# dusk-network/dusk-blindbidproof

Measured on AMD Instinct MI355X. Metric: blind-bid proofs/sec, higher is better.
Workload: dtype u32

## Files before the change

dusk_blindbidproof_amd/csrc/capi_prove.hip:

```cpp
#include <stdio.h>
#include <string.h>
#include <unistd.h>

#include <algorithm>
#include <chrono>
#include <functional>
#include <thread>

#include "batch.h"
#include "chacha.h"
#include "round_bids.h"
#include "submit.h"
#include "witness_check.h"

namespace bbp {
int32_t prove_batch_dev(bbp_ctx* ctx, u32 B, u32 N, const u8* in_dev, const u8* ent_dev, u8* out_dev, hipStream_t s,
                        const std::function<int32_t(hipStream_t)>* open_hook = nullptr);
int32_t verify_batch_dev(bbp_ctx* ctx, const VerifyRows& v, u32 G, const u8* in_dev, const u8* ent_dev, int32_t* status_dev, hipStream_t s);
int32_t verify_batch_agg_dev(bbp_ctx* ctx, const VerifyRows& v, u32 G, const u8* in_dev, const u8* ent_dev, int32_t* status_dev, hipStream_t s,
                             u32* n_fallback, u32* total_out_dev = nullptr);
int32_t debug_read_misc(bbp_ctx* ctx, u32 B, u32 N, u32 proof, uint8_t* out);
int32_t debug_varbase(bbp_ctx* ctx, u32 form, u32 B, u32 Q, u32 agg, const u32* ns, const u8* vers, const u8* pts, const u8* scal, const u8* wv,
                      const u8* uj, u8* sums_out, u32* digits_out, int32_t* status_out);
int32_t round_consts_launch(bbp_ctx* ctx, u32 N, const u8* round_dev, const u32* roff_dev, sc* rblk, int32_t* rflag, hipStream_t s);
// ... 1338 lines not shown
                rcs[i] = bbp_reserve(ctx->members[i], max_batch, N);
            }
        }
        for (auto& t : th) t.join();
        for (int32_t r : rcs)
            if (r) return r;
        return BBP_OK;
    }
    return no_throw_ctx(ctx, [&]() -> int32_t {
        const uint32_t B = max_batch;
        const VerifyRows vrows = VerifyRows::uniform(B, N);
        std::vector<uint8_t> in(prove_in_bytes(N) * B, 0), ent(entropy_row_bytes(N) * B, 0), out(proof_record_bytes(N) * B), vin(vrows.row_bytes(0) * B, 0);
        std::vector<int32_t> st(B);
        int32_t rc = BBP_OK;
        for (int k = 0; k < bbp_ctx::IO_SLOTS && rc == BBP_OK; k++) rc = prove_batch_host(ctx, B, N, in.data(), ent.data(), out.data(), st.data(), CHECK_OFF);
        const uint32_t small = B < 1023 ? B : 1023;
        for (int k = 0; k < bbp_ctx::PROVE_BUFS && rc == BBP_OK; k++) rc = prove_batch_host(ctx, small, N, in.data(), ent.data(), out.data(), st.data(), CHECK_OFF);
        if (B >= 1024 && ctx->knobs.deep_eligible(B)) {
            struct Reset { bool& b; ~Reset() { b = false; } } reset{ctx->prove_state.force_deep};
            ctx->prove_state.force_deep = true;
            for (int k = 0; k < bbp_ctx::PROVE_BUFS && rc == BBP_OK; k++) rc = prove_batch_host(ctx, B, N, in.data(), ent.data(), out.data(), st.data(), CHECK_OFF);
        }
        for (int k = 0; k < bbp_ctx::IO_VSLOTS && rc == BBP_OK; k++) rc = verify_batch_host(ctx, vrows, vin.data(), st.data());
        const bool check = ctx->prove_check;
        for (int k = 0; check && k < bbp_ctx::IO_VSLOTS && rc == BBP_OK; k++) rc = verify_batch_host(ctx, vrows, vin.data(), st.data(), BBP_AGG_GROUP_DEFAULT);
        if (rc == BBP_OK)
            rc = api_guard(ctx, [&]() -> int32_t {
                int32_t rc = BBP_OK;
                BBP_HIP_TRY(ctx, hipSetDevice(ctx->device));
                for (int k = 0; k < bbp_ctx::IO_SLOTS && rc == BBP_OK; k++)
                    if (!(rc = staging_reserve(ctx, ctx->io[k], ProveStaging(B, N, true, check, false)))) rc = staging_reserve(ctx, ctx->io[k], ProveStaging(B, N, false, check, false));
                for (int k = 0; k < bbp_ctx::CHECK_RING && rc == BBP_OK; k++)
                    if (!(rc = dev_reserve(ctx, ctx->rnd[k].buf, RoundRing(B, N, true).bytes)) && check) rc = dev_reserve(ctx, ctx->chk[k].buf, CheckRing(B, N).bytes);
                return rc;
            });
        return rc;
    });
}

extern "C" int32_t bbp_set_batching(bbp_ctx* ctx, uint32_t window_us, uint32_t max_batch) {
    if (!ctx || !ctx->combiner) return BBP_ERR_BAD_ARG;
    return no_throw([&]() -> int32_t {
        static_cast<Combiner*>(ctx->combiner)->configure(window_us, max_batch);
        return BBP_OK;
    });
}

extern "C" int32_t bbp_set_verify_mixing(bbp_ctx* ctx, int32_t on) {
    if (!ctx || !ctx->combiner) return BBP_ERR_BAD_ARG;
    return no_throw([&]() -> int32_t {
        static_cast<Combiner*>(ctx->combiner)->set_verify_mixing(on != 0);
        return BBP_OK;
    });
}

extern "C" int32_t bbp_set_verify_round_sharing(bbp_ctx* ctx, int32_t on) {
    if (!ctx || !ctx->combiner) return BBP_ERR_BAD_ARG;
    return no_throw([&]() -> int32_t {
        static_cast<Combiner*>(ctx->combiner)->set_round_sharing(on != 0);
        return BBP_OK;
    });
}

extern "C" int32_t bbp_verify_round_sharing_stats(bbp_ctx* ctx, uint64_t* n_calls, uint64_t* n_rows, uint64_t* n_rounds) {
    if (!ctx || !ctx->combiner) return BBP_ERR_BAD_ARG;
    return no_throw([&]() -> int32_t {
// ... 105 lines not shown
```

dusk_blindbidproof_amd/csrc/context.h:

```cpp
#pragma once
#include <hip/hip_runtime.h>
#include <stdint.h>
#include <stdio.h>
#include <stdlib.h>
#include <string.h>

#include <atomic>
#include <condition_variable>
#include <map>
#include <mutex>
#include <new>
#include <stdexcept>
#include <string>
#include <vector>

#include "../../include/bbp.h"
#include "point.h"
#include "msm_plan.h"
#include "prove_io.h"
#include "prove_plan.h"
#include "scalar.h"
#include "verify_rows.h"

namespace bbp {
// ... 100 lines not shown
            size_t cap = 0;
            hipEvent_t ev = nullptr;
        };
        std::vector<NsStage> ns_ring;
        uint32_t ns_oldest = 0;
    };
    VLane vl[VLANES];
    std::string err;
    bbp::u32* health = nullptr;
    std::atomic<int> prove_check{0};
    std::atomic<uint64_t> chk_checked{0}, chk_reproved{0};
    unsigned long long* chk_counts = nullptr;
    int64_t debug_corrupt_proof = -1;
    uint32_t chk_lane = 0;
    hipEvent_t ev_chk_fork = nullptr, ev_chk_join = nullptr;
    static constexpr int CHECK_RING = PROVE_BUFS;
    struct CheckBuf {
        bbp::DevBuf buf;
        hipEvent_t ev = nullptr;
        bool ev_valid = false;
    };
    CheckBuf chk[CHECK_RING];
    uint32_t chk_next = 0;
    CheckBuf rnd[CHECK_RING];
    uint32_t rnd_next = 0;
    hipEvent_t ev_round = nullptr;
    bbp::ge* gens = nullptr;
    bbp::niels_row* ptable = nullptr;
    bbp::ge* btab = nullptr;
    bbp::niels_packed* comb = nullptr;
    bbp::sc* mimc_c = nullptr;
    uint8_t gens_enc_host_valid = 0;
    std::vector<uint8_t> mimc_host;
    bbp::DevBuf scal, idx, sorted, pts, enc, batch[PROVE_BUFS + VLANES], io_in, io_out, io_ent, raw[2];
    static constexpr int VERIFY_SLOT = MAX_SLICES;
    bbp::DevBuf slice_sorted[MAX_SLICES + VLANES], slice_pts[MAX_SLICES + VLANES], slice_fold[MAX_SLICES], slice_vtab[MAX_SLICES];
    struct IoSlot {
        bbp::DevBuf in, ent, out, chk;
        uint32_t* h_flag = nullptr;
        void *h_out = nullptr, *h_in = nullptr;
        size_t h_cap = 0, h_in_cap = 0;
        hipEvent_t ev = nullptr, ev_in = nullptr;
        bool busy = false;
    };
    static constexpr int IO_SLOTS = 3;
    static constexpr int IO_VSLOTS = VLANES;
    IoSlot io[IO_SLOTS + IO_VSLOTS];
    std::mutex io_mu;
    std::condition_variable io_cv;
    uint32_t io_next = 0, io_vnext = 0;
    std::map<uint32_t, void*> circuits;
    void* vctab = nullptr;
    uint8_t vctab_has[256] = {};
    std::map<uint64_t, bbp::u32*> layout_idx;
    std::vector<float> timings;
    uint64_t scratch_allocs = 0;
    size_t scratch_bytes = 0;
    bool profile = false;
    struct Ev {
        int tag;
        hipEvent_t a, b;
    };
    std::vector<Ev> events;
};

namespace bbp {

// ... 180 lines not shown
```

dusk_blindbidproof_amd/csrc/prove_plan.h:

```cpp
#pragma once
#include <stdint.h>
#include <stdio.h>
#include <stdlib.h>
#include <string.h>

#include <string>

namespace bbp {

constexpr int FOLD_ROUND = 7;
constexpr int PROVE_MAX_SLICES = 4;
#ifndef BBP_PROVE_BUFS
#define BBP_PROVE_BUFS 5
#endif
constexpr int PROVE_BUFS = BBP_PROVE_BUFS;

struct ProveKnobs {
    int slices = 3;
    int rotate_below = 1023;
    int rotate_deep_max = 4096;
    int deep_from = 3;
    int mixed_from = 512;
    int dual_open_below = 1024;
    int rng_coop = -1;
    int rng_coop_below = 768;
    int rng_coop_idle_below = 2300;
    int rng_dpp = 2;
    int rng_block = 0;
    int serial_block = 64;
    int serial_lds = 160 * 1024;
    int tr_wave_below = 32;
    int ipa_wide_below = 32;
    int commit_split_below = 1024;
    int witness_native = 1;
    int tail_small_below = 65;
    int tail_round = FOLD_ROUND;
    int stagger_mode = 0;
    int trace_prove = 0;

    struct Env {
        const char* name;
        int ProveKnobs::*member;
        int (*clamp)(int);
    };
    template <class F>
    static void each_env(F&& f) {
        static const Env table[] = {
            {"BBP_SLICES", &ProveKnobs::slices, [](int v) { return v < 1 ? 1 : v > PROVE_MAX_SLICES ? PROVE_MAX_SLICES : v; }},
            {"BBP_ROTATE_BELOW", &ProveKnobs::rotate_below, nullptr},
            {"BBP_ROTATE_DEEP_MAX", &ProveKnobs::rotate_deep_max, nullptr},
            {"BBP_ROTATE_DEEP_FROM", &ProveKnobs::deep_from, [](int v) { return v < 2 ? 2 : v; }},
            {"BBP_ROTATE_MIXED_FROM", &ProveKnobs::mixed_from, nullptr},
            {"BBP_DUAL_OPEN_BELOW", &ProveKnobs::dual_open_below, nullptr},
            {"BBP_RNG_COOP", &ProveKnobs::rng_coop, [](int v) { return v != 0 ? 1 : 0; }},
            {"BBP_RNG_COOP_BELOW", &ProveKnobs::rng_coop_below, nullptr},
            {"BBP_RNG_COOP_IDLE_BELOW", &ProveKnobs::rng_coop_idle_below, nullptr},
            {"BBP_RNG_DPP", &ProveKnobs::rng_dpp, nullptr},
            {"BBP_RNG_BLOCK", &ProveKnobs::rng_block, [](int v) { return v >= 1024 ? 1024 : v >= 512 ? 512 : v >= 256 ? 256 : v >= 128 ? 128 : 64; }},
            {"BBP_SERIAL_BLOCK", &ProveKnobs::serial_block, [](int v) { return v == 64 ? 64 : v == 128 ? 128 : 256; }},
            {"BBP_SERIAL_LDS", &ProveKnobs::serial_lds, [](int v) { return v < 0 ? 0 : v > 160 * 1024 ? 160 * 1024 : v; }},
            {"BBP_TR_WAVE_BELOW", &ProveKnobs::tr_wave_below, nullptr},
            {"BBP_IPA_WIDE_BELOW", &ProveKnobs::ipa_wide_below, nullptr},
            {"BBP_COMMIT_SPLIT_BELOW", &ProveKnobs::commit_split_below, nullptr},
            {"BBP_WITNESS_NATIVE", &ProveKnobs::witness_native, [](int v) { return v != 0 ? 1 : 0; }},
            {"BBP_TAIL_SMALL_BELOW", &ProveKnobs::tail_small_below, nullptr},
            {"BBP_TAIL_ROUND", &ProveKnobs::tail_round, [](int v) { return v == FOLD_ROUND ? FOLD_ROUND : 12; }},
            {"BBP_STAGGER", &ProveKnobs::stagger_mode, nullptr},
            {"BBP_TRACE_PROVE", &ProveKnobs::trace_prove, [](int) { return 1; }},
        };
        for (const Env& e : table) f(e);
    }
    bool set(const char* name, const char* text) {
        bool found = false;
        each_env([&](const Env& e) {
            if (strcmp(e.name, name)) return;
            this->*e.member = e.clamp ? e.clamp(atoi(text)) : atoi(text);
            found = true;
        });
        return found;
    }
    static ProveKnobs from_env() {
        ProveKnobs k;
        each_env([&](const Env& e) {
            if (const char* text = getenv(e.name)) k.set(e.name, text);
        });
        return k;
    }

    bool deep_eligible(uint32_t B) const { return slices > 1 && rotate_deep_max > 0 && B <= (uint32_t)rotate_deep_max; }
    unsigned lds_token() const { return serial_lds >= 160 * 1024 ? 64u : 0u; }
};

struct ProveRuleState {
    bool deep_mode = false;
    int deep_idle_seen = 0;
    bool force_deep = false;
    bool last_sliced = false;
    uint32_t calls = 0;
};

struct HeavyPlan {
    uint32_t tw = 0;
    uint32_t tgrid = 0;
    bool wide_ipa = false;
    bool split_T = false;
    uint32_t tail_from = 12;
    int stagger_after = 0;
};

inline HeavyPlan plan_heavy(const ProveKnobs& k, uint32_t B) {
    HeavyPlan h;
    h.tw = B <= (uint32_t)k.tr_wave_below ? 1u : 0u;
    h.tgrid = h.tw ? B : (B + 63) / 64;
    h.wide_ipa = B <= (uint32_t)k.ipa_wide_below;
    h.split_T = B * 5 <= (uint32_t)k.commit_split_below;
    h.tail_from = B < (uint32_t)(k.tail_small_below > 0 ? k.tail_small_below : 0) ? 12u : (uint32_t)k.tail_round;
    h.stagger_after = k.stagger_mode;
    return h;
}

struct ProvePlan {
    enum Chain { SERIAL, LANES25, WORD, HALFWORD };
    uint32_t call = 0;
    bool deep = false;
    bool behind_sliced = false;
    bool dual = false;
    int open_stream = 0;
    int par = 0;
    bool coop = false;
    Chain chain = SERIAL;
    uint32_t prefix_form = 0;
    uint32_t serial_blk = 64;
    uint32_t cblk = 64;
    bool rotate = false;
    int heavy_stream = 0;
    uint32_t slices = 0;

    uint32_t cblk_wave() const { return 2 * cblk > 1024u ? 1024u : 2 * cblk; }
    uint32_t slice_first(uint32_t B, uint32_t i) const { return (uint32_t)(((uint64_t)B * i) / slices); }

    std::string trace_line(uint32_t call_, uint32_t B, int inflight) const {
        char buf[160];
        snprintf(buf, sizeof buf, "prove call %u: B %u inflight %d deep %d behind_sliced %d dual %d rotate %d par %d coop %d\n", call_, B, inflight,
                 (int)deep, (int)behind_sliced, (int)dual, (int)rotate, par, (int)coop);
        return buf;
    }
};

template <class Busy>
ProvePlan plan_prove(const ProveKnobs& k, ProveRuleState& st, uint32_t B, int inflight, Busy&& sliced_busy) {
    ProvePlan p;
    p.call = st.calls++;
    if (inflight >= k.deep_from) {
        st.deep_mode = true;
        st.deep_idle_seen = 0;
    } else if (++st.deep_idle_seen >= 6) {
        st.deep_mode = false;
    }
    p.deep = (st.deep_mode || st.force_deep) && k.deep_eligible(B);
    p.behind_sliced = !p.deep && k.mixed_from > 0 && B >= (uint32_t)k.mixed_from && st.last_sliced && sliced_busy();
    p.dual = !p.behind_sliced && (p.deep || B < (uint32_t)(k.dual_open_below > 0 ? k.dual_open_below : 0));
    p.open_stream = p.dual ? (int)(p.call & 1u) : 0;
    p.par = p.dual ? (int)(p.call % (uint32_t)PROVE_BUFS) : (int)(p.call & 1u);
    p.coop = k.rng_coop < 0 ? B <= (uint32_t)k.rng_coop_below || (inflight == 0 && B <= (uint32_t)k.rng_coop_idle_below) : k.rng_coop != 0;
    p.chain = !p.coop ? ProvePlan::SERIAL : k.rng_dpp >= 2 ? ProvePlan::HALFWORD : k.rng_dpp ? ProvePlan::WORD : ProvePlan::LANES25;
    p.prefix_form = !p.coop ? 0u : B <= (uint32_t)k.tr_wave_below ? 2u : 1u;
    p.serial_blk = k.serial_lds > 0 ? (uint32_t)k.serial_block : 64u;
    p.cblk = k.rng_block > 0 ? (uint32_t)k.rng_block : (B <= 128 ? 64u : B <= 256 ? 128u : 256u);
    p.rotate = p.dual && ((k.rotate_below > 0 && B <= (uint32_t)k.rotate_below) || (p.deep && B > (uint32_t)k.rotate_below));
    p.heavy_stream = p.rotate ? 1 + (int)(p.call % (uint32_t)(PROVE_MAX_SLICES - 1)) : 0;
    p.slices = B >= 64u * (uint32_t)k.slices ? (uint32_t)k.slices : (B >= 128 ? 2u : 1u);
    if (p.dual && p.slices > 2) p.slices = 2;
    if (p.rotate) p.slices = 0;
    return p;
}

}
```

dusk_blindbidproof_amd/csrc/prover.hip:

```cpp
#define BBP_KECCAK_WAVE 1
#include <string.h>

#include <functional>

#include "batch.h"
#include "hosthash.h"
#include "keccak_wave.h"
#include "scalarmul.h"
#include "witness.h"

namespace bbp {

#define BBP_THIN_PRIO() __builtin_amdgcn_s_setprio(3)
#ifndef BBP_LANE_KERNEL
#define BBP_LANE_KERNEL __launch_bounds__(64)
#endif


__device__ __forceinline__ void sc_to_bytes32(uint8_t* o, const sc& s) { sc_tobytes(o, s); }
__device__ __forceinline__ void words_to_bytes32(uint8_t* o, const u32* w) {
#pragma unroll
    for (int i = 0; i < 8; i++) {
        o[4 * i] = (uint8_t)w[i];
        o[4 * i + 1] = (uint8_t)(w[i] >> 8);
// ... 1178 lines not shown
    bd.r1 = (sc*)(base + o_r1); bd.r3 = (sc*)(base + o_r3); bd.a = (sc*)(base + o_a); bd.b = (sc*)(base + o_b); bd.g = (sc*)(base + o_g);
    bd.h = (sc*)(base + o_h); bd.lr = (sc*)(base + o_lr); bd.pts = (ge*)(base + o_pts); bd.lrpts = (ge*)(base + o_lrpts); bd.fpts = (ge*)(base + o_fpts);
    bd.enc = (u32*)(base + o_enc); bd.entropy = base + o_ent;
    return BBP_OK;
}

static merlin_transcript prover_prefix() {
    merlin_transcript t;
    merlin_init(t, reinterpret_cast<const uint8_t*>("BlindBidProofGadget"), 19);
    merlin_append(t, reinterpret_cast<const uint8_t*>("dom-sep"), 7, reinterpret_cast<const uint8_t*>("r1cs v1"), 7);
    return t;
}

#define LAUNCH_LDS(ctx, tag, kern, grid, block, lds, stream, ...)                        \
    do {                                                                                 \
        ScopedEvent _ev(ctx, tag, stream);                                               \
        hipLaunchKernelGGL(kern, dim3(grid), dim3(block), lds, stream, __VA_ARGS__);     \
        BBP_HIP_TRY(ctx, hipGetLastError());                                             \
    } while (0)
#define LAUNCH(ctx, tag, kern, grid, block, stream, ...) LAUNCH_LDS(ctx, tag, kern, grid, block, lds_token(ctx), stream, __VA_ARGS__)

static inline u32 cdiv(u32 a, u32 b) { return (a + b - 1) / b; }

int32_t tail_btab_build(bbp_ctx* ctx) {
    BBP_HIP_TRY(ctx, hipMalloc(&ctx->btab, sizeof(ge) * TAIL_TAB));
    hipLaunchKernelGGL(k_tail_tables, dim3(1), dim3(64), 0, ctx->stream, 1u, ctx->gens + BBP_BASE_B, ctx->btab);
    BBP_HIP_TRY(ctx, hipGetLastError());
    return BBP_OK;
}

size_t tail_btab_bytes() { return sizeof(ge) * TAIL_TAB; }

static BatchDev batch_view(const BatchDev& bd, const CircuitDev& c, u32 first);
static int32_t prove_heavy(bbp_ctx* ctx, const HeavyPlan& hp, const CircuitDev& c, const BatchDev& bd, u32 B, u8* out_dev, hipStream_t s, int slot,
                           hipEvent_t stagger, hipEvent_t out_guard);

int32_t prove_batch_dev(bbp_ctx* ctx, u32 B, u32 N, const u8* in_dev, const u8* ent_dev, u8* out_dev, hipStream_t s,
                        const std::function<int32_t(hipStream_t)>* open_hook) {
    const CircuitDev* cp;
    int32_t rc = circuit_get(ctx, N, &cp);
    if (rc) return rc;
    const CircuitDev& c = *cp;
    StreamGuard guard(ctx, s);
    if ((rc = guard.enter())) return rc;
    int inflight = 0;
    for (int k = 0; k < bbp_ctx::CALL_RING; k++)
        if (ctx->ev_call_valid[k] && hipEventQuery(ctx->ev_call[k]) == hipErrorNotReady) inflight++;
    const ProvePlan plan = plan_prove(ctx->knobs, ctx->prove_state, B, inflight, [&] {
        const int lp = ctx->last_prove_par;
        return lp >= 0 && ctx->ev_done_valid[lp] && hipEventQuery(ctx->ev_done[lp]) == hipErrorNotReady;
    });
    const int sidx = plan.open_stream, par = plan.par;
    if (plan.dual && !ctx->side2) BBP_HIP_TRY(ctx, hipStreamCreateWithFlags(&ctx->side2, hipStreamNonBlocking));
    BatchDev bd;
    if ((rc = batch_reserve(ctx, B, c, bd, par))) return rc;
    const u32 m = c.m, n1 = c.n_mul, encw = (m + 8 + 22) * 8;
    const merlin_transcript prefix = prover_prefix();
    const size_t n_draws = 3 + 2 * (size_t)n1;
    if ((rc = dev_reserve(ctx, ctx->raw[sidx], (size_t)B * n_draws * 64))) return rc;
    u32* const raw = (u32*)ctx->raw[sidx].p;
    BBP_HIP_TRY(ctx, hipEventRecord(ctx->ev_entry[par], s));
    hipStream_t os = sidx ? ctx->side2 : ctx->side;
    if (ctx->ev_done_valid[par]) BBP_HIP_TRY(ctx, hipStreamWaitEvent(os, ctx->ev_done[par], 0));
    if (ctx->ev_prep_valid) {
        BBP_HIP_TRY(ctx, hipStreamWaitEvent(os, ctx->ev_prep, 0));
        ctx->ev_prep_valid = false;
    }
    if (ctx->ev_draw_valid) {
        BBP_HIP_TRY(ctx, hipStreamWaitEvent(os, ctx->ev_draw, 0));
        ctx->ev_draw_valid = false;
    }
    if (open_hook && (rc = (*open_hook)(os))) return rc;
    LAUNCH(ctx, TAG_WITNESS, k_fill_mimc, cdiv(B * BBP_MIMC_ROUNDS, 64), 64, os, B, c.n_cst, ctx->mimc_c, bd.cst);
    u32 hog = 0;
    if ((rc = serial_lds_bytes(ctx, (const void*)k_open_serial, &hog))) return rc;
    LAUNCH(ctx, TAG_WITNESS, k_witness_head, cdiv(B, 64), 64, os, B, N, c.n_cst, in_dev, bd.cst, bd.v);
    LAUNCH(ctx, TAG_TRANSCRIPT, k_load_blindings, cdiv(B * m, 64), 64, os, B, m, ent_dev, bd.vb);
    if ((rc = commit_launch(ctx, B * m, bd.v, bd.vb, m, m, m, bd.pts, m + 8, os))) return rc;
    LAUNCH(ctx, TAG_ENCODE, k_encode_strided, cdiv(B * m, 64), 64, os, B * m, m, bd.pts, m + 8, bd.enc, encw, 0u, 1u);
    if (plan.coop) {
        const u32 pgrid = plan.prefix_form == 2 ? B : cdiv(B, 64);
        LAUNCH(ctx, TAG_RNG, k_open_serial, pgrid, 64, os, B, pgrid, m, n1, prefix, bd.enc, ent_dev, bd.vb, raw, bd.tr, bd.rng, c.n_cst, c.w_terms,
               c.w_loff, c.w_roff, bd.cst, bd.v, bd.ai1, bd.ao1, plan.prefix_form);
    }
    auto bulk = [&](decltype(&k_open_bulk) kern, u32 lanes, u32 blk) -> int32_t {
        u32 hogb = 0;
        if (int32_t rc = serial_lds_bytes(ctx, (const void*)kern, &hogb)) return rc;
        const u32 nb_rng = cdiv(B * lanes, blk), nb_wit = cdiv(B, blk);
        LAUNCH_LDS(ctx, TAG_RNG, kern, nb_rng + nb_wit, blk, hogb, os, B, nb_rng, n1, 2 + 2 * n1, bd.rng, raw, m, c.n_cst, c.w_terms, c.w_loff,
                   c.w_roff, bd.cst, bd.v, bd.ai1, bd.ao1, hogb, (u32)ctx->knobs.witness_native);
        return BBP_OK;
    };
    switch (plan.chain) {
        case ProvePlan::SERIAL:
            LAUNCH_LDS(ctx, TAG_RNG, k_open_serial, 2 * cdiv(B, plan.serial_blk), plan.serial_blk, hog, os, B, cdiv(B, plan.serial_blk), m, n1, prefix,
                       bd.enc, ent_dev, bd.vb, raw, bd.tr, bd.rng, c.n_cst, c.w_terms, c.w_loff, c.w_roff, bd.cst, bd.v, bd.ai1, bd.ao1, 0u);
            break;
        case ProvePlan::LANES25: rc = bulk(k_open_bulk, 32, plan.cblk); break;
        case ProvePlan::WORD: rc = bulk(k_open_bulk8, 64, plan.cblk_wave()); break;
        case ProvePlan::HALFWORD: rc = bulk(k_open_bulk50, 64, plan.cblk_wave()); break;
    }
    if (rc) return rc;
    LAUNCH(ctx, TAG_RNG, k_reduce_draws, cdiv((u32)(B * n_draws), 128), 128, os, B, n1, (const u32*)raw, bd.ai1, bd.ao1, bd.s1,
           plan.chain == ProvePlan::HALFWORD ? 1u : 0u);
    BBP_HIP_TRY(ctx, hipEventRecord(ctx->ev_open[par], os));
    ctx->ev_open_valid[par] = true;
    if (ctx->knobs.trace_prove) fputs(plan.trace_line(plan.call, B, inflight).c_str(), stderr);
    const size_t rec = BBP_R1CS_PROOF_BYTES + 32 * (size_t)m;
    if (plan.rotate) {
        const int hs = plan.heavy_stream;
        hipStream_t ls = ctx->lane[hs];
        BBP_HIP_TRY(ctx, hipStreamWaitEvent(ls, ctx->ev_open[par], 0));
        if ((rc = prove_heavy(ctx, plan_heavy(ctx->knobs, B), c, bd, B, out_dev, ls, hs, nullptr, ctx->ev_entry[par]))) return rc;
        BBP_HIP_TRY(ctx, hipEventRecord(ctx->ev_join[hs], ls));
        BBP_HIP_TRY(ctx, hipStreamWaitEvent(s, ctx->ev_join[hs], 0));
    }
    for (u32 i = 0; i < plan.slices; i++) {
        const u32 first = plan.slice_first(B, i), last = plan.slice_first(B, i + 1);
        hipStream_t ls = i == 0 ? s : ctx->lane[i];
        BBP_HIP_TRY(ctx, hipStreamWaitEvent(ls, ctx->ev_open[par], 0));
        const HeavyPlan hp = plan_heavy(ctx->knobs, last - first);
        if (i && hp.stagger_after) BBP_HIP_TRY(ctx, hipStreamWaitEvent(ls, ctx->ev_stagger[i - 1], 0));
        if ((rc = prove_heavy(ctx, hp, c, batch_view(bd, c, first), last - first, out_dev + rec * first, ls, (int)i,
                              i + 1 < plan.slices ? ctx->ev_stagger[i] : nullptr, i ? ctx->ev_entry[par] : nullptr)))
            return rc;
        if (i) {
            BBP_HIP_TRY(ctx, hipEventRecord(ctx->ev_join[i], ls));
            BBP_HIP_TRY(ctx, hipStreamWaitEvent(s, ctx->ev_join[i], 0));
        }
    }
    BBP_HIP_TRY(ctx, hipEventRecord(ctx->ev_done[par], s));
    ctx->ev_done_valid[par] = true;
    ctx->last_par = par;
    ctx->prove_state.last_sliced = !plan.rotate;
    ctx->last_prove_par = par;
    BBP_HIP_TRY(ctx, hipEventRecord(ctx->ev_call[plan.call % (u32)bbp_ctx::CALL_RING], s));
    ctx->ev_call_valid[plan.call % (u32)bbp_ctx::CALL_RING] = true;
    return BBP_OK;
}

static BatchDev batch_view(const BatchDev& bd, const CircuitDev& c, u32 first) {
    BatchDev v = bd;
    const size_t f = first, n1 = c.n_mul, m = c.m;
    v.cst += f * c.n_cst; v.v += f * m; v.vb += f * m; v.ai1 += f * (1 + 2 * n1); v.ao1 += f * (1 + n1); v.s1 += f * (1 + 2 * n1);
    v.tr += f; v.rng += f; v.misc += f * MS_COUNT; v.zpow += f * ((size_t)c.n_cons + 1); v.ypow += f * 2049; v.yipow += f * 2048;
    v.wl += f * 2048; v.wr += f * 2048; v.wo += f * 2048; v.wv += f * m; v.l1 += f * n1; v.r0 += f * n1; v.r1 += f * n1; v.r3 += f * n1;
    v.a += f * 2048; v.b += f * 2048; v.g += f * 2048; v.h += f * 2048; v.lr += f * 2 * 2049; v.pts += f * (m + 8); v.lrpts += f * 2; v.fpts += f * 2 * FOLD_CLS;
    v.enc += f * (m + 8 + 22) * 8; v.entropy += f * (32 * m + 32);
    return v;
}

static int32_t prove_heavy(bbp_ctx* ctx, const HeavyPlan& hp, const CircuitDev& c, const BatchDev& bd, u32 B, u8* out_dev, hipStream_t s, int slot,
// ... 83 lines not shown
```

dusk_blindbidproof_amd/csrc/setup.hip:

```cpp
#include <stdio.h>
#include <stdlib.h>

#include <dirent.h>
#include <unistd.h>

#include <atomic>
#include <mutex>

#include "context.h"
#include "batch.h"
#include "hosthash.h"
#include "submit.h"

namespace bbp {

__global__ void k_derive_generators(const u32* __restrict__ uniform, ge* __restrict__ gens) {
    u32 i = blockIdx.x * blockDim.x + threadIdx.x;
    if (i > 2 * BBP_GENS_CAPACITY + 1) return;
    if (i == 2 * BBP_GENS_CAPACITY + 1) {
        gens[BBP_BASE_B] = ge_basepoint();
        return;
    }
    u32 w[16];
#pragma unroll
// ... 185 lines not shown
        BBP_HIP_TRY(ctx, hipStreamCreateWithFlags(&ctx->lane[i], hipStreamNonBlocking));
        BBP_HIP_TRY(ctx, hipEventCreateWithFlags(&ctx->ev_join[i], hipEventDisableTiming));
        BBP_HIP_TRY(ctx, hipEventCreateWithFlags(&ctx->ev_stagger[i - 1], hipEventDisableTiming));
    }
    BBP_HIP_TRY(ctx, hipStreamCreateWithFlags(&ctx->copy, hipStreamNonBlocking));
    BBP_HIP_TRY(ctx, hipStreamCreateWithFlags(&ctx->side2, hipStreamNonBlocking));
    for (auto& L : ctx->vl) {
#ifdef BBP_VL_SKIP
        if (&L == &ctx->vl[1])
            for (int k = 0; k < BBP_VL_SKIP; k++) {
                hipStream_t d;
                BBP_HIP_TRY(ctx, hipStreamCreateWithFlags(&d, hipStreamNonBlocking));
                ctx->spare_streams.push_back(d);
            }
#endif
        BBP_HIP_TRY(ctx, hipStreamCreateWithFlags(&L.stream, hipStreamNonBlocking));
        BBP_HIP_TRY(ctx, hipEventCreateWithFlags(&L.ev_vfork, hipEventDisableTiming));
        BBP_HIP_TRY(ctx, hipEventCreateWithFlags(&L.ev_vjoin, hipEventDisableTiming));
    }
    for (int f = 0; f < bbp_ctx::FAMILIES; f++) BBP_HIP_TRY(ctx, hipEventCreateWithFlags(&ctx->ev_last[f], hipEventDisableTiming));
    for (auto& sl : ctx->io) {
        BBP_HIP_TRY(ctx, hipHostMalloc((void**)&sl.h_flag, sizeof(uint32_t), hipHostMallocDefault));
        *sl.h_flag = 0;
        BBP_HIP_TRY(ctx, hipEventCreateWithFlags(&sl.ev, hipEventDisableTiming));
        BBP_HIP_TRY(ctx, hipEventCreateWithFlags(&sl.ev_in, hipEventDisableTiming));
    }
    BBP_HIP_TRY(ctx, hipEventCreateWithFlags(&ctx->ev_prep, hipEventDisableTiming));
    BBP_HIP_TRY(ctx, hipEventCreateWithFlags(&ctx->ev_draw, hipEventDisableTiming));
    if (const char* e = getenv("BBP_VERIFY_OVERLAP")) ctx->verify_overlap = atoi(e) != 0;
    if (const char* e = getenv("BBP_VERIFY_SERIAL_ACC")) ctx->verify_serial_acc = atoi(e) != 0;
    for (auto& e : ctx->ev_vacc) BBP_HIP_TRY(ctx, hipEventCreateWithFlags(&e, hipEventDisableTiming));
    if (const char* e = getenv("BBP_VERIFY_AGGREGATE")) ctx->verify_group = atoi(e) > 1 ? (uint32_t)atoi(e) : 0u;
    ctx->knobs = ProveKnobs::from_env();
    if (const char* e = getenv("BBP_VARBASE_LANES")) ctx->varbase_lanes = atoi(e) < 64 ? 64 : atoi(e);
    ctx->msm_knobs = MsmKnobs::from_env();
    for (int i = 0; i < bbp_ctx::PROVE_BUFS; i++) {
        BBP_HIP_TRY(ctx, hipEventCreateWithFlags(&ctx->ev_entry[i], hipEventDisableTiming));
        BBP_HIP_TRY(ctx, hipEventCreateWithFlags(&ctx->ev_open[i], hipEventDisableTiming));
        BBP_HIP_TRY(ctx, hipEventCreateWithFlags(&ctx->ev_done[i], hipEventDisableTiming));
    }
    for (auto& e : ctx->ev_call) BBP_HIP_TRY(ctx, hipEventCreateWithFlags(&e, hipEventDisableTiming));

    const size_t n_uniform = 2 * BBP_GENS_CAPACITY + 1;
    std::vector<uint8_t> uniform(n_uniform * 64);
    static const uint8_t B_ENC[32] = {0xe2, 0xf2, 0xae, 0x0a, 0x6a, 0xbc, 0x4e, 0x71, 0xa8, 0x84, 0xa9, 0x61, 0xc5, 0x00, 0x51, 0x5f,
                                      0x58, 0xe3, 0x0b, 0x6a, 0xa5, 0x82, 0xdd, 0x8d, 0xb6, 0xa6, 0x59, 0x45, 0xe0, 0x8d, 0x2d, 0x76};
    sha3_512(B_ENC, 32, &uniform[0]);
    for (int which = 0; which < 2; which++) {
        uint8_t seed[20] = {'G', 'e', 'n', 'e', 'r', 'a', 't', 'o', 'r', 's', 'C', 'h', 'a', 'i', 'n', (uint8_t)(which ? 'H' : 'G'), 0, 0, 0, 0};
        shake256(seed, 20, &uniform[64 * (1 + (size_t)which * BBP_GENS_CAPACITY)], 64 * BBP_GENS_CAPACITY);
    }
    mimc_constants_host(ctx->mimc_host);

    u32* d_uniform = nullptr;
    BBP_HIP_TRY(ctx, hipMalloc(&d_uniform, uniform.size()));
    BBP_HIP_TRY(ctx, hipMemcpyAsync(d_uniform, uniform.data(), uniform.size(), hipMemcpyHostToDevice, ctx->stream));
    BBP_HIP_TRY(ctx, hipMalloc(&ctx->gens, sizeof(ge) * TAB_BASES));
    BBP_HIP_TRY(ctx, hipMalloc(&ctx->ptable, sizeof(niels_row) * (size_t)TAB_BASES * MSM_POS));
    BBP_HIP_TRY(ctx, hipMalloc(&ctx->comb, sizeof(niels_packed) * 2 * 64 * 8));
    BBP_HIP_TRY(ctx, hipMalloc(&ctx->mimc_c, sizeof(sc) * BBP_MIMC_ROUNDS));
    BBP_HIP_TRY(ctx, hipMalloc(&ctx->health, sizeof(u32)));
    BBP_HIP_TRY(ctx, hipMemset(ctx->health, 0, sizeof(u32)));
    BBP_HIP_TRY(ctx, hipMemcpyAsync(ctx->mimc_c, ctx->mimc_host.data(), 32 * BBP_MIMC_ROUNDS, hipMemcpyHostToDevice, ctx->stream));
    hipLaunchKernelGGL(k_derive_generators, dim3((BBP_NUM_BASES + 63) / 64), dim3(64), 0, ctx->stream, d_uniform, ctx->gens);
    BBP_HIP_TRY(ctx, hipGetLastError());
    hipLaunchKernelGGL(k_pad_sums, dim3(1), dim3(64), 0, ctx->stream, ctx->gens);
// ... 1 lines not shown
    hipLaunchKernelGGL(k_merge_sums, dim3(2048 / 64), dim3(64), 0, ctx->stream, ctx->gens);
    BBP_HIP_TRY(ctx, hipGetLastError());
    hipLaunchKernelGGL(k_build_ptable, dim3((TAB_BASES * (MSM_POS / PT_CHUNK) + 63) / 64), dim3(64), 0, ctx->stream, ctx->gens, ctx->ptable);
    BBP_HIP_TRY(ctx, hipGetLastError());
    if (int32_t rc = tail_btab_build(ctx)) return rc;
    hipLaunchKernelGGL(k_build_comb, dim3(2), dim3(64), 0, ctx->stream, ctx->gens, ctx->comb);
    BBP_HIP_TRY(ctx, hipGetLastError());
    BBP_HIP_TRY(ctx, hipStreamSynchronize(ctx->stream));
    BBP_HIP_TRY(ctx, hipFree(d_uniform));
    return BBP_OK;
}

extern "C" void bbp_free(bbp_ctx* ctx) {
    if (!ctx) return;
    if (is_pool(ctx)) {
        delete static_cast<Combiner*>(ctx->combiner);
        ctx->combiner = nullptr;
        pool_workers_stop(ctx);
        for (bbp_ctx* m : ctx->members) bbp_free(m);
        ctx->members.clear();
        delete ctx;
        return;
    }
    if (!ctx->stream && !ctx->gens && ctx->device < 0) {
        delete static_cast<Combiner*>(ctx->combiner);
        delete ctx;
        return;
    }
    delete static_cast<Combiner*>(ctx->combiner);
    ctx->combiner = nullptr;
    (void)hipSetDevice(ctx->device);
    (void)hipDeviceSynchronize();
    std::vector<void*> ptrs = {ctx->gens, ctx->ptable, ctx->btab, ctx->comb, ctx->mimc_c, ctx->scal.p, ctx->idx.p, ctx->sorted.p, ctx->pts.p, ctx->enc.p,
                               ctx->io_in.p, ctx->io_out.p, ctx->io_ent.p, ctx->raw[0].p, ctx->raw[1].p};
    for (auto& b : ctx->batch) ptrs.push_back(b.p);
    for (auto& b : ctx->slice_sorted) ptrs.push_back(b.p);
    for (auto& b : ctx->slice_pts) ptrs.push_back(b.p);
    for (auto& b : ctx->slice_fold) ptrs.push_back(b.p);
    for (auto& b : ctx->slice_vtab) ptrs.push_back(b.p);
    for (void* p : ptrs)
        if (p) (void)hipFree(p);
    for (auto& kv : ctx->circuits) {
        bbp::CircuitDev* c = static_cast<bbp::CircuitDev*>(kv.second);
        if (!c) continue;
        void* cp[] = {c->w_terms, c->w_loff, c->w_roff, c->f_off, c->f_ent, c->c_q, c->c_cst, c->idx_ai, c->idx_s1, c->idx_ao, c->idx_ipa, c->idx_ver};
        for (void* p : cp)
            if (p) (void)hipFree(p);
        delete c;
    }
    ctx->circuits.clear();
    for (auto& sl : ctx->io) {
        for (void* p : {sl.in.p, sl.ent.p, sl.out.p, sl.chk.p})
            if (p) (void)hipFree(p);
        if (sl.h_flag) (void)hipHostFree(sl.h_flag);
        if (sl.h_out) (void)hipHostFree(sl.h_out);
        if (sl.h_in) (void)hipHostFree(sl.h_in);
        if (sl.ev) (void)hipEventDestroy(sl.ev);
        if (sl.ev_in) (void)hipEventDestroy(sl.ev_in);
    }
    if (ctx->vctab) (void)hipFree(ctx->vctab);
    if (ctx->health) (void)hipFree(ctx->health);
    if (ctx->chk_counts) (void)hipFree(ctx->chk_counts);
    for (auto& cb : ctx->chk) {
        if (cb.buf.p) (void)hipFree(cb.buf.p);
        if (cb.ev) (void)hipEventDestroy(cb.ev);
    }
    for (auto& cb : ctx->rnd) {
// ... 70 lines not shown
            off += (uint32_t)snprintf(buf + off, cap - off, "member %zu (worker threads on NUMA node %d): ", i, pool_member_numa_node(ctx, (uint32_t)i));
            if (off + 1 >= cap) break;
            if (int32_t rc = bbp_describe(ctx->members[i], buf + off, cap - off)) return rc;
            off += (uint32_t)strlen(buf + off);
        }
        return BBP_OK;
    }
    return api_guard(ctx, [&]() -> int32_t {
        BBP_HIP_TRY(ctx, hipSetDevice(ctx->device));
        hipDeviceProp_t prop;
        BBP_HIP_TRY(ctx, hipGetDeviceProperties(&prop, ctx->device));
        size_t free_b = 0, total_b = 0;
        BBP_HIP_TRY(ctx, hipMemGetInfo(&free_b, &total_b));
        const char* hwq = getenv("GPU_MAX_HW_QUEUES");
        uint32_t off = (uint32_t)snprintf(buf, cap,
                                          "device %d: %s (%s), %d CUs, %.0f MHz, %.1f of %.1f GiB free; prover: %d heavy-stage slices, tail from round %d, "
                                          "cooperative rng below %d proofs; verifier: %d lanes, accumulates %s, aggregate groups of %u%s\n",
                                          ctx->device, prop.name, prop.gcnArchName, prop.multiProcessorCount, prop.clockRate / 1e3, free_b / 1073741824.0,
                                          total_b / 1073741824.0, ctx->knobs.slices, ctx->knobs.tail_round, ctx->knobs.rng_coop_below, (int)bbp_ctx::VLANES,
                                          ctx->verify_serial_acc ? "chained" : "free-running", ctx->verify_group, ctx->verify_group ? "" : " (off)");
        const int hst = hw_queues_state();
        if (off + 1 < cap)
            off += (uint32_t)snprintf(buf + off, cap - off, "hardware queues: GPU_MAX_HW_QUEUES=%s (%s); scratch: %.2f GiB in %llu allocation(s) since bbp_init\n",
                                      hwq ? hwq : "unset",
                                      hst == 2 ? "exported by the library before HIP initialised" : hst == 1 ? "from the caller's environment" : hst == 3 ? "unset and HIP was already initialised" : "?",
                                      ctx->scratch_bytes / 1073741824.0, (unsigned long long)ctx->scratch_allocs);
        if ((hst == 3 || !hwq || atoi(hwq) < atoi(BBP_HWQ_DEFAULT)) && off + 1 < cap)
            off += (uint32_t)snprintf(buf + off, cap - off,
                                      "WARNING: GPU_MAX_HW_QUEUES is %s%s: the HIP runtime reads it once, when it initialises; export the library's default"
                                      " before the process first touches HIP (or call bbp_init first: it does so itself), or streams of this context share "
                                      "fewer hardware queues and serialise\n",
                                      hwq ? hwq : "not set", hst == 3 ? " and HIP was initialised before bbp_init could set it" : "");
        if (off + 1 < cap)
            off += (uint32_t)snprintf(buf + off, cap - off, "checked proving: %s\n",
                                      ctx->prove_check ? "on (every record is verified on the device before it is returned)" : "off");
        if (off + 1 < cap && ctx->combiner)
            off += (uint32_t)snprintf(buf + off, cap - off, "verify mixing: %s\n",
                                      static_cast<Combiner*>(ctx->owner && ctx->owner->combiner ? ctx->owner->combiner : ctx->combiner)->verify_mixing()
                                          ? "on (concurrent bbp_verify callers share a call whatever their bid-list length)"
                                          : "off (one call per bid-list length and record layout)");
        if (off + 1 < cap && ctx->combiner &&
            static_cast<Combiner*>(ctx->owner && ctx->owner->combiner ? ctx->owner->combiner : ctx->combiner)->round_sharing())
            off += (uint32_t)snprintf(buf + off, cap - off,
                                      "verify round sharing: on (concurrent bbp_verify callers with a byte-equal seed and bid list share one table entry)\n");
        if (off + 1 < cap)
            off += (uint32_t)snprintf(buf + off, cap - off, "entropy source: %s\n",
                                      ctx->entropy_source == BBP_ENTROPY_SOURCE_DEVICE
                                          ? "device (one 32-byte OS key per call, expanded with ChaCha20 on the device)"
                                          : "os (the calling thread reads /dev/urandom and reduces the blindings on the host)");
        if (free_b < ((size_t)6 << 30) && off + 1 < cap)
            off += (uint32_t)snprintf(buf + off, cap - off, "WARNING: less than 6 GiB of device memory free: a 1024-proof batch needs ~14 GiB of scratch\n");
        return BBP_OK;
    });
}

extern "C" int32_t bbp_debug_corrupt_scratch(bbp_ctx* ctx) {
    if (!ctx) return BBP_ERR_BAD_ARG;
    if (is_pool(ctx)) return bbp_debug_corrupt_scratch(ctx->members[0]);
    return api_guard(ctx, [&]() -> int32_t {
        ctx->debug_corrupt = 1;
        return BBP_OK;
    });
}

extern "C" int32_t bbp_check_health(bbp_ctx* ctx, uint32_t* flags) {
    if (!ctx || !flags) return BBP_ERR_BAD_ARG;
// ... 45 lines not shown
```

Measured before the change: 21160.

## Run opening stage on each rotating call's own chain stream when queues are few

For rotating (deep-pipeline) prove calls, the opening stage can now run on the same stream as that call's heavy stage, forming three independent chains on side, lane[1] and lane[2]. Previously openings ran on side/side2 and heavy stages on lane[1..3]. The rule turns on by default when GPU_MAX_HW_QUEUES is below 7, to avoid streams sharing hardware queues and serialising. It adds more raw entropy buffers (four instead of two), pre-reserves them during warmup, and adds extra cross-stream waits on ev_join[3]. These waits could add serialization or ordering hazards if the role mapping is wrong.

```diff
diff --git a/dusk_blindbidproof_amd/csrc/capi_prove.hip b/dusk_blindbidproof_amd/csrc/capi_prove.hip
--- a/dusk_blindbidproof_amd/csrc/capi_prove.hip
+++ b/dusk_blindbidproof_amd/csrc/capi_prove.hip
@@ -1394,6 +1394,12 @@
                     if (!(rc = staging_reserve(ctx, ctx->io[k], ProveStaging(B, N, true, check, false)))) rc = staging_reserve(ctx, ctx->io[k], ProveStaging(B, N, false, check, false));
                 for (int k = 0; k < bbp_ctx::CHECK_RING && rc == BBP_OK; k++)
                     if (!(rc = dev_reserve(ctx, ctx->rnd[k].buf, RoundRing(B, N, true).bytes)) && check) rc = dev_reserve(ctx, ctx->chk[k].buf, CheckRing(B, N).bytes);
+                const CircuitDev* c = nullptr;
+                if (rc == BBP_OK && !(rc = circuit_get(ctx, N, &c))) {
+                    const uint32_t dual_max = std::max((uint32_t)std::max(ctx->knobs.dual_open_below - 1, 0), ctx->knobs.deep_eligible(1) ? (uint32_t)ctx->knobs.rotate_deep_max : 0u);
+                    for (auto& r : ctx->raw)
+                        if (rc == BBP_OK) rc = dev_reserve(ctx, r, (size_t)std::min(B, dual_max) * (3 + 2 * (size_t)c->n_mul) * 64);
+                }
                 return rc;
             });
         return rc;
diff --git a/dusk_blindbidproof_amd/csrc/context.h b/dusk_blindbidproof_amd/csrc/context.h
--- a/dusk_blindbidproof_amd/csrc/context.h
+++ b/dusk_blindbidproof_amd/csrc/context.h
@@ -156,7 +156,7 @@
     bbp::sc* mimc_c = nullptr;
     uint8_t gens_enc_host_valid = 0;
     std::vector<uint8_t> mimc_host;
-    bbp::DevBuf scal, idx, sorted, pts, enc, batch[PROVE_BUFS + VLANES], io_in, io_out, io_ent, raw[2];
+    bbp::DevBuf scal, idx, sorted, pts, enc, batch[PROVE_BUFS + VLANES], io_in, io_out, io_ent, raw[4];
     static constexpr int VERIFY_SLOT = MAX_SLICES;
     bbp::DevBuf slice_sorted[MAX_SLICES + VLANES], slice_pts[MAX_SLICES + VLANES], slice_fold[MAX_SLICES], slice_vtab[MAX_SLICES];
     struct IoSlot {
diff --git a/dusk_blindbidproof_amd/csrc/prove_plan.h b/dusk_blindbidproof_amd/csrc/prove_plan.h
--- a/dusk_blindbidproof_amd/csrc/prove_plan.h
+++ b/dusk_blindbidproof_amd/csrc/prove_plan.h
@@ -37,6 +37,8 @@
     int tail_round = FOLD_ROUND;
     int stagger_mode = 0;
     int trace_prove = 0;
+    int open_on_chain = -1;
+    int hw_queues = 4;
 
     struct Env {
         const char* name;
@@ -67,6 +69,7 @@
             {"BBP_TAIL_ROUND", &ProveKnobs::tail_round, [](int v) { return v == FOLD_ROUND ? FOLD_ROUND : 12; }},
             {"BBP_STAGGER", &ProveKnobs::stagger_mode, nullptr},
             {"BBP_TRACE_PROVE", &ProveKnobs::trace_prove, [](int) { return 1; }},
+            {"BBP_OPEN_ON_CHAIN", &ProveKnobs::open_on_chain, [](int v) { return v < 0 ? -1 : v ? 1 : 0; }},
         };
         for (const Env& e : table) f(e);
     }
@@ -88,6 +91,7 @@
     }
 
     bool deep_eligible(uint32_t B) const { return slices > 1 && rotate_deep_max > 0 && B <= (uint32_t)rotate_deep_max; }
+    bool chain_rule(bool deep) const { return open_on_chain == 1 || (open_on_chain < 0 && deep && hw_queues < 7); }
     unsigned lds_token() const { return serial_lds >= 160 * 1024 ? 64u : 0u; }
 };
 
@@ -119,6 +123,8 @@
     return h;
 }
 
+enum StreamRole { ROLE_CALLER = 0, ROLE_SIDE, ROLE_LANE1, ROLE_LANE2, ROLE_LANE3, ROLE_COPY, ROLE_SIDE2, ROLE_COUNT };
+
 struct ProvePlan {
     enum Chain { SERIAL, LANES25, WORD, HALFWORD };
     uint32_t call = 0;
@@ -135,7 +141,19 @@
     bool rotate = false;
     int heavy_stream = 0;
     uint32_t slices = 0;
+    bool open_on_chain = false;
+    int chain_stream = -1;
 
+    int open_role() const { return open_on_chain ? chain_stream : open_stream ? ROLE_SIDE2 : ROLE_SIDE; }
+    int heavy_role() const { return open_on_chain ? chain_stream : ROLE_LANE1 + heavy_stream - 1; }
+    static int slice_role(uint32_t i) { return i == 0 ? ROLE_CALLER : ROLE_LANE1 + (int)i - 1; }
+    uint32_t roles() const {
+        uint32_t mask = 1u << ROLE_CALLER | 1u << open_role();
+        if (rotate) mask |= 1u << heavy_role();
+        for (uint32_t i = 0; i < slices; i++) mask |= 1u << slice_role(i);
+        return mask;
+    }
+    int raw_index() const { return !open_on_chain ? open_stream : chain_stream == ROLE_SIDE ? 0 : 1 + heavy_stream; }
     uint32_t cblk_wave() const { return 2 * cblk > 1024u ? 1024u : 2 * cblk; }
     uint32_t slice_first(uint32_t B, uint32_t i) const { return (uint32_t)(((uint64_t)B * i) / slices); }
 
@@ -172,6 +190,8 @@
     p.slices = B >= 64u * (uint32_t)k.slices ? (uint32_t)k.slices : (B >= 128 ? 2u : 1u);
     if (p.dual && p.slices > 2) p.slices = 2;
     if (p.rotate) p.slices = 0;
+    p.open_on_chain = p.rotate && k.chain_rule(p.deep);
+    p.chain_stream = !p.open_on_chain ? -1 : p.heavy_stream == 3 ? (int)ROLE_SIDE : (int)ROLE_LANE1 + p.heavy_stream - 1;
     return p;
 }
 
diff --git a/dusk_blindbidproof_amd/csrc/prover.hip b/dusk_blindbidproof_amd/csrc/prover.hip
--- a/dusk_blindbidproof_amd/csrc/prover.hip
+++ b/dusk_blindbidproof_amd/csrc/prover.hip
@@ -1234,6 +1234,17 @@
 size_t tail_btab_bytes() { return sizeof(ge) * TAIL_TAB; }
 
 static BatchDev batch_view(const BatchDev& bd, const CircuitDev& c, u32 first);
+static hipStream_t role_stream(bbp_ctx* ctx, int role, hipStream_t caller) {
+    switch (role) {
+        case ROLE_CALLER: return caller;
+        case ROLE_SIDE: return ctx->side;
+        case ROLE_SIDE2: return ctx->side2;
+        case ROLE_LANE1: return ctx->lane[1];
+        case ROLE_LANE2: return ctx->lane[2];
+        case ROLE_LANE3: return ctx->lane[3];
+        default: return nullptr;
+    }
+}
 static int32_t prove_heavy(bbp_ctx* ctx, const HeavyPlan& hp, const CircuitDev& c, const BatchDev& bd, u32 B, u8* out_dev, hipStream_t s, int slot,
                            hipEvent_t stagger, hipEvent_t out_guard);
 
@@ -1252,17 +1263,18 @@
         const int lp = ctx->last_prove_par;
         return lp >= 0 && ctx->ev_done_valid[lp] && hipEventQuery(ctx->ev_done[lp]) == hipErrorNotReady;
     });
-    const int sidx = plan.open_stream, par = plan.par;
-    if (plan.dual && !ctx->side2) BBP_HIP_TRY(ctx, hipStreamCreateWithFlags(&ctx->side2, hipStreamNonBlocking));
+    const int ridx = plan.raw_index(), par = plan.par;
+    if (plan.open_role() == ROLE_SIDE2 && !ctx->side2) BBP_HIP_TRY(ctx, hipStreamCreateWithFlags(&ctx->side2, hipStreamNonBlocking));
     BatchDev bd;
     if ((rc = batch_reserve(ctx, B, c, bd, par))) return rc;
     const u32 m = c.m, n1 = c.n_mul, encw = (m + 8 + 22) * 8;
     const merlin_transcript prefix = prover_prefix();
     const size_t n_draws = 3 + 2 * (size_t)n1;
-    if ((rc = dev_reserve(ctx, ctx->raw[sidx], (size_t)B * n_draws * 64))) return rc;
-    u32* const raw = (u32*)ctx->raw[sidx].p;
+    if ((rc = dev_reserve(ctx, ctx->raw[ridx], (size_t)B * n_draws * 64))) return rc;
+    u32* const raw = (u32*)ctx->raw[ridx].p;
     BBP_HIP_TRY(ctx, hipEventRecord(ctx->ev_entry[par], s));
-    hipStream_t os = sidx ? ctx->side2 : ctx->side;
+    hipStream_t os = role_stream(ctx, plan.open_role(), s);
+    if (plan.chain_stream == ROLE_SIDE) BBP_HIP_TRY(ctx, hipStreamWaitEvent(os, ctx->ev_join[3], 0));
     if (ctx->ev_done_valid[par]) BBP_HIP_TRY(ctx, hipStreamWaitEvent(os, ctx->ev_done[par], 0));
     if (ctx->ev_prep_valid) {
         BBP_HIP_TRY(ctx, hipStreamWaitEvent(os, ctx->ev_prep, 0));
@@ -1311,15 +1323,17 @@
     const size_t rec = BBP_R1CS_PROOF_BYTES + 32 * (size_t)m;
     if (plan.rotate) {
         const int hs = plan.heavy_stream;
-        hipStream_t ls = ctx->lane[hs];
-        BBP_HIP_TRY(ctx, hipStreamWaitEvent(ls, ctx->ev_open[par], 0));
+        hipStream_t ls = role_stream(ctx, plan.heavy_role(), s);
+        if (!plan.open_on_chain) BBP_HIP_TRY(ctx, hipStreamWaitEvent(ls, ctx->ev_open[par], 0));
+        if (!plan.open_on_chain && hs == 3) BBP_HIP_TRY(ctx, hipStreamWaitEvent(ls, ctx->ev_join[3], 0));
         if ((rc = prove_heavy(ctx, plan_heavy(ctx->knobs, B), c, bd, B, out_dev, ls, hs, nullptr, ctx->ev_entry[par]))) return rc;
         BBP_HIP_TRY(ctx, hipEventRecord(ctx->ev_join[hs], ls));
         BBP_HIP_TRY(ctx, hipStreamWaitEvent(s, ctx->ev_join[hs], 0));
     }
     for (u32 i = 0; i < plan.slices; i++) {
         const u32 first = plan.slice_first(B, i), last = plan.slice_first(B, i + 1);
-        hipStream_t ls = i == 0 ? s : ctx->lane[i];
+        hipStream_t ls = role_stream(ctx, ProvePlan::slice_role(i), s);
+        if (i == 3) BBP_HIP_TRY(ctx, hipStreamWaitEvent(ls, ctx->ev_join[3], 0));
         BBP_HIP_TRY(ctx, hipStreamWaitEvent(ls, ctx->ev_open[par], 0));
         const HeavyPlan hp = plan_heavy(ctx->knobs, last - first);
         if (i && hp.stagger_after) BBP_HIP_TRY(ctx, hipStreamWaitEvent(ls, ctx->ev_stagger[i - 1], 0));
diff --git a/dusk_blindbidproof_amd/csrc/setup.hip b/dusk_blindbidproof_amd/csrc/setup.hip
--- a/dusk_blindbidproof_amd/csrc/setup.hip
+++ b/dusk_blindbidproof_amd/csrc/setup.hip
@@ -241,6 +241,7 @@
     for (auto& e : ctx->ev_vacc) BBP_HIP_TRY(ctx, hipEventCreateWithFlags(&e, hipEventDisableTiming));
     if (const char* e = getenv("BBP_VERIFY_AGGREGATE")) ctx->verify_group = atoi(e) > 1 ? (uint32_t)atoi(e) : 0u;
     ctx->knobs = ProveKnobs::from_env();
+    if (const char* e = getenv("GPU_MAX_HW_QUEUES")) ctx->knobs.hw_queues = atoi(e) > 0 ? atoi(e) : 4;
     if (const char* e = getenv("BBP_VARBASE_LANES")) ctx->varbase_lanes = atoi(e) < 64 ? 64 : atoi(e);
     ctx->msm_knobs = MsmKnobs::from_env();
     for (int i = 0; i < bbp_ctx::PROVE_BUFS; i++) {
@@ -308,7 +309,8 @@
     (void)hipSetDevice(ctx->device);
     (void)hipDeviceSynchronize();
     std::vector<void*> ptrs = {ctx->gens, ctx->ptable, ctx->btab, ctx->comb, ctx->mimc_c, ctx->scal.p, ctx->idx.p, ctx->sorted.p, ctx->pts.p, ctx->enc.p,
-                               ctx->io_in.p, ctx->io_out.p, ctx->io_ent.p, ctx->raw[0].p, ctx->raw[1].p};
+                               ctx->io_in.p, ctx->io_out.p, ctx->io_ent.p};
+    for (auto& b : ctx->raw) ptrs.push_back(b.p);
     for (auto& b : ctx->batch) ptrs.push_back(b.p);
     for (auto& b : ctx->slice_sorted) ptrs.push_back(b.p);
     for (auto& b : ctx->slice_pts) ptrs.push_back(b.p);
@@ -445,6 +447,12 @@
                                       "fewer hardware queues and serialise\n",
                                       hwq ? hwq : "not set", hst == 3 ? " and HIP was initialised before bbp_init could set it" : "");
         if (off + 1 < cap)
+            off += (uint32_t)snprintf(buf + off, cap - off, "rotating prove calls: opening stage %s (BBP_OPEN_ON_CHAIN %s, schedule fitted to %d hardware queue(s))\n",
+                                      ctx->knobs.chain_rule(false) ? "on the call's own chain stream: three chains on side, lane[1], lane[2]"
+                                      : ctx->knobs.chain_rule(true) ? "on the call's own chain stream for the calls of a deep pipeline (three chains on side, lane[1], lane[2]), else on side / side2"
+                                                                    : "on side / side2, heavy stage on lane[1..3]",
+                                      ctx->knobs.open_on_chain < 0 ? "unset: deep pipelines below 7 queues" : ctx->knobs.open_on_chain ? "= 1" : "= 0", ctx->knobs.hw_queues);
+        if (off + 1 < cap)
             off += (uint32_t)snprintf(buf + off, cap - off, "checked proving: %s\n",
                                       ctx->prove_check ? "on (every record is verified on the device before it is returned)" : "off");
         if (off + 1 < cap && ctx->combiner)
```

New measurement: 22270 (median of 6 runs). +5.3%, better.
